# volume-em/empanada

Measured on AMD Instinct MI355X. Metric: Mvox/s end-to-end 3D panoptic inference (incl. consensus); PQ vs CPU ref, higher is better.
Workload: dtype f32

## Files before the change

### empanada_amd/_hip.py

```python
import ctypes
import os

import torch

_HERE = os.path.dirname(os.path.abspath(__file__))
LIB_PATH = os.path.join(_HERE, 'libemp_hip.so')

MAX_KS = 11
MAX_CLASSES = 16
MAX_CENTERS = 4096
CENTER_LIMIT = 65535


class HipError(RuntimeError):
    pass


_c = ctypes
_P = _c.c_void_p
_I = _c.c_int
_L = _c.c_int64
_F = _c.c_float
_U32 = _c.c_uint32

SIGNATURES = {
    'emp_version': (_I, []),
    'emp_last_error': (_c.c_char_p, []),
    'emp_device_count': (_I, []),
    'emp_bn_act_nhwc': (_I, [_P, _P, _P, _P, _I, _L, _I, _P, _L, _P]),
    'emp_dwconv_nhwc': (_I, [_P, _P, _P, _I, _I, _I, _I, _I, _P, _P]),
    'emp_upsample_bilinear': (_I, [_P, _I, _I, _I, _I, _P, _P, _I, _I, _P, _P]),
    'emp_conv_bn_act_proj_nhwc': (_I, [_P, _P, _P, _P, _I] + [_I] * 10 + [_P, _I, _P, _P, _L, _P]),
    'emp_conv_k_slab': (_I, [_L, _I, _I, _I]),
    'emp_conv_k_slab_cin': (_I, [_L, _I, _I, _I, _I]),
    'emp_conv_k_slab_geom': (_I, [_L, _I, _I, _I, _I, _I, _I, _I, _I]),
    'emp_conv1x1_ws_eligible': (_I, [_L, _I, _I, _I, _I, _I, _I, _I]),
    'emp_gconv_chunk': (_I, [_I]),
    'emp_gconv3x3_bn_act_nhwc': (_I, [_P, _L, _P, _P, _P, _I, _I, _I, _I, _I, _I, _I, _P, _L, _P]),
    'emp_conv_bn_act_nhwc': (_I, [_P, _P, _P, _P, _P, _L, _I] + [_I] * 10 + [_P, _L, _P]),
    'emp_conv_splitk_plan': (_I, [_L, _I, _I, _I, _I]),
    'emp_conv_splitk_bn_act_nhwc': (_I, [_P, _P, _P, _P, _P, _L, _I] + [_I] * 11 + [_P, _P, _L, _P]),
    'emp_wino_input_transform': (_I, [_P, _I, _I, _I, _I, _I, _P, _L, _P, _P]),
    'emp_gemm_nt_batched': (_I, [_P, _P, _I, _L, _I, _I, _P, _P]),
    'emp_wino4_input_transform': (_I, [_P, _I, _I, _I, _I, _I, _P, _L, _P, _P]),
    'emp_wino4_output_transform': (_I, [_P, _P, _L, _I, _I, _I, _I, _I, _P, _P, _I, _P, _L, _P]),
    'emp_wino4_conv_bn_act_nhwc': (_I, [_P, _I, _I, _I, _I, _I, _P, _L, _P, _I, _P, _P, _I, _P, _L, _P]),
    'emp_wino4_fused_eligible': (_I, [_L, _I, _I, _I]),
    'emp_wino3_input_transform': (_I, [_P, _I, _I, _I, _I, _I, _P, _L, _P, _P]),
    'emp_wino3_output_transform': (_I, [_P, _P, _L, _I, _I, _I, _I, _I, _P, _P, _I, _P, _L, _P]),
    'emp_wino_gemm_fused': (_I, [_P, _I, _I, _I, _I, _I, _P, _L, _P, _I, _P, _P]),
    'emp_wino_output_transform': (_I, [_P, _P, _L, _I, _I, _I, _I, _I, _P, _P, _I, _P, _L, _P]),
    'emp_chain_class': (_I, [_L, _P, _P, _P, _I, _P, _P, _P, _P, _L, _L, _c.c_double, _c.c_double, _P, _P, _P, _P]),
    'emp_lsap_maximize': (_L, [_P, _L, _L, _P, _P]),
    'emp_slices_to_input': (_I, [_P, _L, _L, _L, _I, _I, _I, _I, _I, _F, _F, _P, _P]),
    'emp_slices_to_input_scaled': (_I, [_P, _L, _L, _L] + [_I] * 7 + [_P, _P, _P, _P, _I, _F, _F, _P, _P]),
    'emp_pointwise_out_nhwc': (_I, [_P, _P, _P, _L, _L, _I, _I, _P, _P]),
    'emp_bn_relu_maxpool_nhwc': (_I, [_P, _P, _P, _I, _I, _I, _I, _P, _P]),
    'emp_stem_conv7_bn_relu_maxpool': (_I, [_P, _P, _P, _P, _I, _I, _I, _P, _P]),
    'emp_logits_to_prob': (_I, [_P, _I, _I, _L, _P, _P]),
    'emp_upsample_bilinear_prob': (_I, [_P, _I, _I, _I, _I, _P, _P, _I, _I, _P, _I, _P]),
    'emp_pr_upsample2x': (_I, [_P, _I, _I, _I, _I, _P, _P, _P]),
    'emp_pr_topk_work_bytes': (_L, [_I, _L]),
    'emp_pr_topk': (_I, [_P, _I, _L, _I, _P, _L, _P, _P]),
    'emp_pr_point_sample': (_I, [_P, _L, _P, _I, _I, _I, _I, _I, _P, _I, _I, _I, _P, _P, _I, _P]),
    'emp_pr_scatter': (_I, [_P, _I, _P, _I, _I, _I, _L, _P, _P]),
    'emp_median_harden_stack': (_I, [_P, _I, _I, _L, _I, _F, _P, _P, _P]),
    'emp_median_step': (_I, [_c.POINTER(_P), _I, _L, _P, _P]),
    'emp_harden': (_I, [_P, _I, _I, _L, _F, _P, _P]),
    'emp_find_centers': (_I, [_P, _I, _I, _I, _F, _I, _I, _P, _P, _P]),
    'emp_find_centers_work_elems': (_L, [_I, _I, _I, _I]),
    'emp_find_centers_ws': (_I, [_P, _I, _I, _I, _F, _I, _I, _P, _P, _P, _P]),
    'emp_group_work_elems': (_L, [_I, _I]),
    'emp_group_pixels': (_I, [_P, _P, _I, _P, _I, _I, _I, _I, _P, _U32, _P, _P, _P]),
    'emp_fuse_work_elems': (_L, [_I, _I, _I]),
    'emp_fuse_panoptic': (_I, [_P, _P, _I, _I, _I, _I, _I, _I, _U32, _L, _L, _L, _P, _P, _P, _P]),
    'emp_fuse_lut': (_I, [_P, _P, _I, _I, _I, _I, _I, _I, _U32, _L, _L, _P, _P]),
    'emp_fuse_apply': (_I, [_P, _P, _I, _I, _I, _I, _I, _I, _U32, _L, _L, _P, _P, _P, _P]),
    'emp_runs_count': (_I, [_P, _I, _I, _I, _P, _P]),
    'emp_scan_tmp_elems': (_L, [_L]),
    'emp_exclusive_scan_i32': (_I, [_P, _L, _P, _P, _P]),
    'emp_runs_extract': (_I, [_P, _I, _I, _I, _P, _P, _P, _P, _P]),
    'emp_runs_label_work_elems': (_L, [_L]),
    'emp_runs_label': (_I, [_P, _P, _P, _P, _L, _I, _I, _I, _L, _U32, _P, _P, _P, _P, _P, _P, _P, _P, _P]),
    'emp_runs_overlap_next': (_I, [_P, _P, _P, _P, _P, _L, _I, _I, _I, _L, _P, _L, _P, _P]),
    'emp_rle_decode': (_I, [_P, _P, _P, _L, _P, _P]),
# ... 854 lines not shown
    g = w_oihw.detach().double().cpu()

    def comb(a, b, c):
        return [(G[0] * a + G[1] * b) + G[2] * c for G in _WINO3_G]

    rows = comb(g[:, :, 0, :], g[:, :, 1, :], g[:, :, 2, :])
    U = []
    for r in rows:
        U.extend(comb(r[:, :, 0], r[:, :, 1], r[:, :, 2]))
    return torch.stack(U, dim=0).float().contiguous()


def wino3_conv_bn_act(x, U, tiles_dev, dil, scale=None, shift=None, relu=False, out=None):
    require_gpu()
    N, Cin, H, W = x.shape
    Cout = U.shape[1]
    assert x.is_cuda and x.dtype == torch.float32 and x.is_contiguous(memory_format=torch.channels_last)
    T = tiles_dev.shape[0]
    V = torch.empty((25, T, Cin), dtype=torch.float32, device=x.device)
    Mw = torch.empty((25, T, Cout), dtype=torch.float32, device=x.device)
    if out is None:
        out = torch.empty((N, Cout, H, W), dtype=torch.float32, device=x.device, memory_format=torch.channels_last)
    assert out.shape == (N, Cout, H, W) and out.stride(1) == 1
    ops = out.stride(3)
    assert out.stride(2) == W * ops and out.stride(0) == H * W * ops, "NHWC channel slice required"
    st = stream()
    call('emp_wino3_input_transform', x.data_ptr(), N, H, W, Cin, dil, _ptr(tiles_dev), T, _ptr(V), st,
         alg_bytes=4 * (x.numel() + V.numel()))
    call('emp_gemm_nt_batched', _ptr(V), _ptr(U), 25, T, Cout, Cin, _ptr(Mw), st,
         alg_bytes=4 * (V.numel() + U.numel() + Mw.numel()), alg_flops=2 * 25 * T * Cout * Cin)
    call('emp_wino3_output_transform', _ptr(Mw), _ptr(tiles_dev), T, N, H, W, Cout, dil, _ptr(scale), _ptr(shift),
         int(bool(relu)), out.data_ptr(), ops, st, alg_bytes=4 * (Mw.numel() + N * Cout * H * W))
    return out


def conv_bn_act_proj_nhwc(x, w_okkc, scale, shift, relu, proj_w, proj_b=None, stride=1, pad=0, dil=1, keep=False):
    require_gpu()
    N, Cin, H, W = x.shape
    Cout, KH, KW, _ = w_okkc.shape
    n = proj_w.shape[0]
    assert x.is_cuda and x.dtype == torch.float32 and x.is_contiguous(memory_format=torch.channels_last)
    OH = (H + 2 * pad - dil * (KH - 1) - 1) // stride + 1
    OW = (W + 2 * pad - dil * (KW - 1) - 1) // stride + 1
    acc = torch.zeros((N, n, OH, OW), dtype=torch.float32, device=x.device)
    act = (torch.empty((N, Cout, OH, OW), dtype=torch.float32, device=x.device, memory_format=torch.channels_last)
           if keep else None)
    call('emp_conv_bn_act_proj_nhwc', x.data_ptr(), _ptr(w_okkc), _ptr(scale), _ptr(shift), int(bool(relu)), N, H, W,
         Cin, Cout, KH, KW, stride, pad, dil, _ptr(proj_w), n, _ptr(acc), act.data_ptr() if keep else None, 0,
         stream(), alg_bytes=4 * (x.numel() + w_okkc.numel() + acc.numel() + (act.numel() if keep else 0)),
         alg_flops=2 * N * OH * OW * Cout * (Cin * KH * KW + n))
    if proj_b is not None:
        acc += proj_b.view(1, -1, 1, 1)
    return (acc, act) if keep else acc
```

### empanada_amd/build.py

```python
import os
import subprocess
import sys

HERE = os.path.dirname(os.path.abspath(__file__))
CSRC = os.path.join(HERE, 'csrc')
SOURCES = ['emp_pixel.hip', 'emp_runs.hip', 'emp_ranges.hip', 'emp_tracks.hip', 'emp_dense.hip', 'emp_conv.hip', 'emp_conv1x1.hip', 'emp_wino4.hip', 'emp_gconv.hip', 'emp_stem.hip', 'emp_pointrend.hip', 'emp_chain.cpp']
LIB = os.path.join(HERE, 'libemp_hip.so')
FLAGS = ['--offload-arch=gfx950', '-O3', '-ffp-contract=off', '-fPIC', '-std=c++17', '-Wno-unused-value',
         '-Wno-unused-result', '-Wno-inline-asm']


def _stale(target, deps):
    if not os.path.exists(target):
        return True
    t = os.path.getmtime(target)
    return any(os.path.getmtime(d) > t for d in deps)


def build(force=False, verbose=True):
    hipcc = os.environ.get('HIPCC', 'hipcc')
    headers = [os.path.join(CSRC, 'emp_common.h'), os.path.join(CSRC, 'emp_wino4.h'), os.path.join(HERE, '..', 'include', 'emp_hip.h')]
    objs = []
    for src in SOURCES:
        s = os.path.join(CSRC, src)
        o = os.path.join(CSRC, os.path.splitext(src)[0] + '.o')
        if force or _stale(o, [s] + headers):
            cmd = [hipcc] + FLAGS + ['-c', s, '-o', o]
            if verbose:
                print(' '.join(cmd), flush=True)
            subprocess.run(cmd, check=True)
        objs.append(o)
    if force or _stale(LIB, objs):
        cmd = [hipcc, '--offload-arch=gfx950', '-shared', '-fPIC', '-o', LIB] + objs
        if verbose:
            print(' '.join(cmd), flush=True)
        subprocess.run(cmd, check=True)
    return LIB


if __name__ == '__main__':
    build(force='--force' in sys.argv)
```

### empanada_amd/csrc/emp_conv.hip

```cpp
#include "emp_common.h"
#include "emp_wino4.h"
#include <stdlib.h>

typedef float f32x16 __attribute__((ext_vector_type(16)));

#define CG_BM 128
#define CG_BK 32
#define CG_THREADS 256

struct ConvGeom {
    const float *x, *w, *scale, *shift, *res;
    float *out;
    int N, H, W, Cin, OH, OW, Cout, KH, KW, stride, pad, dil, relu;
    int64_t M, out_ps, res_ps;
    int tiles_m, tiles_n;
    int64_t x_bs, w_bs, out_bs;
    const int32_t *tiles;
    const float *proj_w;
    float *proj_out;
    int proj_n;
    int64_t hw;
};

__device__ __attribute__((aligned(16))) float cg_zero_page[64];
// ... 653 lines not shown
    const int T = g.tiles_m * g.tiles_n;
    const dim3 grid(8 * ((T + 7) / 8), 1, k_splits);
    hipStream_t st = emp_stream(stream);
    if (pl.narrow)
        hipLaunchKernelGGL((conv_igemm_f32_kernel<1, 0, false, 32, false, true>), grid, dim3(CG_THREADS), 0, st, g);
    else
        hipLaunchKernelGGL((conv_igemm_f32_kernel<2, 0, false, 32, false, true>), grid, dim3(CG_THREADS), 0, st, g);
    EMP_CHECK_LAUNCH("emp_conv_splitk_bn_act_nhwc(partials)");
    const int64_t total = g.M * (Cout / 4);
    hipLaunchKernelGGL(splitk_reduce_kernel, dim3(emp_grid(total, 256, 4096)), dim3(256), 0, st, work, k_splits, g.M, Cout,
                       scale, shift, residual, res_pixel_stride, relu, out, out_pixel_stride);
    EMP_CHECK_LAUNCH("emp_conv_splitk_bn_act_nhwc(reduce)");
    return EMP_OK;
}

extern "C" int emp_conv_bn_act_proj_nhwc(const float *x, const float *w_okkc, const float *scale, const float *shift,
                                         int relu, int N, int H, int W, int Cin, int Cout, int KH, int KW, int stride,
                                         int pad, int dil, const float *proj_w, int proj_n, float *proj_out,
                                         float *out, int64_t out_pixel_stride, void *stream)
{
    EMP_REQUIRE(x && w_okkc && proj_w && proj_out, "conv_proj: null pointer");
    EMP_REQUIRE(N >= 0 && H > 0 && W > 0 && Cin > 0 && Cin % CG_BK == 0, "conv_proj: bad shape (Cin %% %d)", CG_BK);
    EMP_REQUIRE(Cout == 128 || Cout == 256, "conv_proj: Cout %d must be 128 or 256 (at most two cout tiles)", Cout);
    EMP_REQUIRE(proj_n >= 1 && proj_n <= 4, "conv_proj: proj_n %d not in 1..4", proj_n);
    EMP_REQUIRE(KH >= 1 && KW >= 1 && KH <= 7 && KW <= 7 && stride >= 1 && dil >= 1 && pad >= 0, "conv_proj: bad filter geometry");
    const int OH = (H + 2 * pad - dil * (KH - 1) - 1) / stride + 1;
    const int OW = (W + 2 * pad - dil * (KW - 1) - 1) / stride + 1;
    EMP_REQUIRE(OH > 0 && OW > 0, "conv_proj: empty output");
    if (out_pixel_stride == 0) out_pixel_stride = Cout;
    EMP_REQUIRE(((reinterpret_cast<uintptr_t>(x) | reinterpret_cast<uintptr_t>(w_okkc) | reinterpret_cast<uintptr_t>(proj_w) |
                  reinterpret_cast<uintptr_t>(out)) & 15) == 0 && (out_pixel_stride & 3) == 0, "conv_proj: alignment");
    EMP_REQUIRE(out != x, "conv_proj: output cannot alias the input");
    if (N == 0) return EMP_OK;
    ConvGeom g;
    g.x = x; g.w = w_okkc; g.scale = scale; g.shift = shift; g.res = nullptr; g.out = out;
    g.N = N; g.H = H; g.W = W; g.Cin = Cin; g.OH = OH; g.OW = OW; g.Cout = Cout; g.KH = KH; g.KW = KW;
    g.stride = stride; g.pad = pad; g.dil = dil; g.relu = relu;
    g.M = (int64_t)N * OH * OW; g.out_ps = out_pixel_stride; g.res_ps = Cout;
    g.x_bs = g.w_bs = g.out_bs = 0; g.tiles = nullptr;
    g.proj_w = proj_w; g.proj_out = proj_out; g.proj_n = proj_n; g.hw = (int64_t)OH * OW;
    const CgPlan pl = cg_plan(g.M, Cout, 1, false, true, false);
    g.tiles_m = pl.tiles_m;
    g.tiles_n = pl.tiles_n;
    const int T = g.tiles_m * g.tiles_n;
    const int grid = 8 * ((T + 7) / 8);
#define CG_GOP(BK_, GL_) hipLaunchKernelGGL((conv_igemm_f32_kernel<2, 0, false, BK_, true, GL_>), dim3(grid), dim3(CG_THREADS), 0, emp_stream(stream), g)
    if (pl.glds) { if (pl.slab == 16) CG_GOP(16, true); else CG_GOP(32, true); }
    else { if (pl.slab == 16) CG_GOP(16, false); else CG_GOP(32, false); }
#undef CG_GOP
    EMP_CHECK_LAUNCH("emp_conv_bn_act_proj_nhwc");
    return EMP_OK;
}


__global__ __launch_bounds__(256) void wino_input_kernel(const float *__restrict__ x, const int32_t *__restrict__ tiles,
                                                         int64_t T, int H, int W, int C4, int dil, float4 *__restrict__ V)
{
    const int64_t total = T * C4;
    for (int64_t i = (int64_t)blockIdx.x * blockDim.x + threadIdx.x; i < total; i += (int64_t)gridDim.x * blockDim.x) {
        const int c4 = (int)(i % C4);
        const int64_t t = i / C4;
        const int n = tiles[3 * t], by = tiles[3 * t + 1], bx = tiles[3 * t + 2];
        const float4 *src = reinterpret_cast<const float4 *>(x) + (int64_t)n * H * W * C4 + c4;
        float4 d[4][4];
#pragma unroll
        for (int a = 0; a < 4; ++a)
#pragma unroll
            for (int b = 0; b < 4; ++b) {
                const int yy = by + a * dil, xx = bx + b * dil;
                d[a][b] = make_float4(0.f, 0.f, 0.f, 0.f);
                if (yy >= 0 && yy < H && xx >= 0 && xx < W) d[a][b] = src[((int64_t)yy * W + xx) * C4];
            }
#define W_SUB(p, q) make_float4(__fsub_rn(p.x, q.x), __fsub_rn(p.y, q.y), __fsub_rn(p.z, q.z), __fsub_rn(p.w, q.w))
#define W_ADD(p, q) make_float4(__fadd_rn(p.x, q.x), __fadd_rn(p.y, q.y), __fadd_rn(p.z, q.z), __fadd_rn(p.w, q.w))
        float4 tt[4][4];
#pragma unroll
        for (int a = 0; a < 4; ++a) {
            tt[a][0] = W_SUB(d[a][0], d[a][2]);
            tt[a][1] = W_ADD(d[a][1], d[a][2]);
            tt[a][2] = W_SUB(d[a][2], d[a][1]);
            tt[a][3] = W_SUB(d[a][1], d[a][3]);
        }
        float4 *dst = V + t * C4 + c4;
        const int64_t ps = T * C4;
#pragma unroll
        for (int v = 0; v < 4; ++v) {
            dst[(0 * 4 + v) * ps] = W_SUB(tt[0][v], tt[2][v]);
            dst[(1 * 4 + v) * ps] = W_ADD(tt[1][v], tt[2][v]);
            dst[(2 * 4 + v) * ps] = W_SUB(tt[2][v], tt[1][v]);
            dst[(3 * 4 + v) * ps] = W_SUB(tt[1][v], tt[3][v]);
        }
    }
}

__global__ __launch_bounds__(256) void wino_output_kernel(const float4 *__restrict__ Mw, const int32_t *__restrict__ tiles,
                                                          int64_t T, int H, int W, int Co4, int dil,
                                                          const float4 *__restrict__ scale, const float4 *__restrict__ shift,
                                                          int relu, float *__restrict__ out, int64_t out_ps)
{
    const int64_t total = T * Co4;
    for (int64_t i = (int64_t)blockIdx.x * blockDim.x + threadIdx.x; i < total; i += (int64_t)gridDim.x * blockDim.x) {
        const int c4 = (int)(i % Co4);
        const int64_t t = i / Co4;
        const int n = tiles[3 * t], oy = tiles[3 * t + 1] + dil, ox = tiles[3 * t + 2] + dil;
        const float4 *src = Mw + t * Co4 + c4;
        const int64_t ps = T * Co4;
// ... 385 lines not shown
```

### empanada_amd/models/panoptic_deeplab.py

```python
import zlib
from typing import List

import torch
import torch.nn as nn
import torch.nn.functional as F

__all__ = ['PanopticDeepLab', 'PanopticDeepLabPR', 'PointRendSemSegHead', 'resnet_encoder', 'prepare_for_inference',
           'tune_fused_convs',
           'synthesize_weights']

_RESNETS = {
    'resnet18': ('basic', [2, 2, 2, 2]), 'resnet34': ('basic', [3, 4, 6, 3]),
    'resnet50': ('bottleneck', [3, 4, 6, 3]), 'resnet101': ('bottleneck', [3, 4, 23, 3]),
    'resnet152': ('bottleneck', [3, 8, 36, 3]),
}


def _conv_bn_act(nin, nout, k, stride=1, groups=1, act=True):
    layers = [nn.Conv2d(nin, nout, k, stride=stride, padding=(k - 1) // 2, groups=groups, bias=False),
              nn.BatchNorm2d(nout)]
    if act:
        layers.append(nn.ReLU(inplace=True))
    return nn.Sequential(*layers)


class SeparableConv2d(nn.Module):

    def __init__(self, nin, nout, kernel_size=3, stride=1, bias=True):
        super().__init__()
        self.sepconv = nn.Sequential(
            nn.Conv2d(nin, nin, kernel_size, stride=stride, padding=(kernel_size - 1) // 2, groups=nin, bias=bias),
            nn.Conv2d(nin, nout, 1, stride=1, bias=bias))

    def forward(self, x):
        return self.sepconv(x)


def _sepconv_bn_act(nin, nout, k):
    return nn.Sequential(SeparableConv2d(nin, nout, k, 1, bias=False), nn.BatchNorm2d(nout), nn.ReLU(inplace=True))


def _bn_affine(bn):
    scale = (bn.weight.detach().float() / torch.sqrt(bn.running_var.detach().float() + bn.eps)).contiguous()
    shift = (bn.bias.detach().float() - bn.running_mean.detach().float() * scale).contiguous()
    return scale, shift


def _no_late_weights(state_dict, prefix, *args):
    raise RuntimeError("load_state_dict after prepare_for_inference: load the weights into the plain model first "
                       f"(module {prefix.rstrip('.')!r} holds folded copies)")


class DepthwiseConvNHWC(nn.Module):

    def __init__(self, conv):
        super().__init__()
        k = conv.kernel_size[0]
        C = conv.in_channels
        self.register_buffer('w_kkc', conv.weight.detach().float().reshape(C, k * k).t().contiguous())
        self.register_buffer('b', conv.bias.detach().float().contiguous() if conv.bias is not None else None)
        self.k = k

    @staticmethod
    def eligible(m):
        return (isinstance(m, nn.Conv2d) and m.groups == m.in_channels == m.out_channels and m.in_channels % 4 == 0
                and m.kernel_size[0] == m.kernel_size[1] and m.kernel_size[0] in (3, 5) and m.stride == (1, 1)
                and m.dilation == (1, 1) and m.padding == (m.kernel_size[0] // 2,) * 2
                and m.padding_mode == 'zeros')

    def forward(self, x):
        from .. import _hip
        if not x.is_contiguous(memory_format=torch.channels_last):
            x = x.contiguous(memory_format=torch.channels_last)
        return _hip.dwconv_nhwc(x, self.w_kkc, self.b, self.k)


class FusedBNAct(nn.Module):

    def __init__(self, bn, relu):
        super().__init__()
        scale, shift = _bn_affine(bn)
        self.register_buffer('scale', scale, persistent=False)
        self.register_buffer('shift', shift, persistent=False)
        self.relu = relu
        self._register_load_state_dict_pre_hook(_no_late_weights)

    def forward(self, x, residual=None, out=None):
        from .. import _hip
# ... 331 lines not shown
        return self.project(torch.cat([conv(x) for conv in self.convs], dim=1))


class PanopticDeepLabDecoder(nn.Module):

    def __init__(self, in_channels, decoder_channels, low_level_stages, low_level_channels,
                 low_level_channels_project, atrous_rates, aspp_channels=None, aspp_dropout=0.5):
        super().__init__()
        aspp_channels = aspp_channels or decoder_channels
        self.aspp = ASPP(in_channels, aspp_channels, atrous_rates, aspp_dropout)
        self.low_level_stages = list(low_level_stages)
        project, fuse = [], []
        for i, (lc, pc) in enumerate(zip(low_level_channels, low_level_channels_project)):
            project.append(_conv_bn_act(lc, pc, 1))
            fuse.append(_sepconv_bn_act((aspp_channels if i == 0 else decoder_channels) + pc, decoder_channels, 5))
        self.project = nn.ModuleList(project)
        self.fuse = nn.ModuleList(fuse)
        self.hip_ops = False

    def forward(self, pyramid: List[torch.Tensor]):
        x = self.aspp(pyramid[-1])
        for stage, proj, fuse in zip(self.low_level_stages, self.project, self.fuse):
            feat = pyramid[stage]
            if self.hip_ops and _can_write_into(proj, feat):
                cx = x.shape[1]
                cl = (proj[0].conv if isinstance(proj[0], FusedConvBNAct) else proj[0]).out_channels
                buf = torch.empty((x.shape[0], cx + cl, feat.shape[2], feat.shape[3]), dtype=x.dtype,
                                  device=x.device, memory_format=torch.channels_last)
                _up_bilinear(x, feat.shape[2:], True, out=buf[:, :cx])
                _conv_bn_into(proj, feat, buf[:, cx:])
                x = fuse(buf)
            else:
                low = proj(feat)
                x = _up_bilinear(x, low.shape[2:], self.hip_ops)
                x = fuse(torch.cat((x, low), dim=1))
        return x


class PanopticDeepLabHead(nn.Module):

    def __init__(self, nin, n_classes):
        super().__init__()
        self.head = nn.Sequential(_sepconv_bn_act(nin, nin, 5), nn.Conv2d(nin, n_classes, 1, bias=True))
        self.hip_ops = False

    def forward(self, x):
        if self.hip_ops and x.is_cuda and x.dtype == torch.float32:
            sep = self.head[0][0]
            site = sep.sepconv[1] if isinstance(sep, SeparableConv2d) else None
            last = self.head[1]
            if (isinstance(site, FusedConvBNAct) and site.impl == 'direct' and isinstance(last, PointwiseOutNHWC)
                    and site.conv.out_channels in (128, 256) and site.conv.kernel_size == (1, 1)):
                from .. import _hip
                y = sep.sepconv[0](x)
                if not y.is_contiguous(memory_format=torch.channels_last):
                    y = y.contiguous(memory_format=torch.channels_last)
                site._prepare('direct')
                return _hip.conv_bn_act_proj_nhwc(y, site._w_okkc, site.bn.scale, site.bn.shift, site.bn.relu,
                                                  last.w, last.b)
        return self.head(x)


class PanopticDeepLab(nn.Module):

    def __init__(self, encoder='resnet50', num_classes=1, stage4_stride=16, decoder_channels=256,
                 low_level_stages=(3, 2, 1), low_level_channels_project=(128, 64, 32), atrous_rates=(2, 4, 6),
                 aspp_channels=None, aspp_dropout=0.1, ins_decoder=False, ins_ratio=0.5, **kwargs):
        super().__init__()
        assert encoder in _RESNETS, f'Invalid encoder name {encoder}, choices are {sorted(_RESNETS)}'
        assert stage4_stride in (16, 32) and min(low_level_stages) > 0
        self.decoder_channels = decoder_channels
        self.num_classes = num_classes
        self.encoder = resnet_encoder(encoder, output_stride=stage4_stride)
        sem_p, ins_p = (aspp_dropout, aspp_dropout) if isinstance(aspp_dropout, float) else aspp_dropout
        widths = self.encoder.cfg.widths
        low_ch = [int(widths[i - 1]) for i in low_level_stages]
        self.semantic_decoder = PanopticDeepLabDecoder(int(widths[-1]), decoder_channels, low_level_stages, low_ch,
                                                       list(low_level_channels_project), atrous_rates,
                                                       aspp_channels, sem_p)
        if ins_decoder:
            self.instance_decoder = PanopticDeepLabDecoder(
                int(widths[-1]), decoder_channels, low_level_stages, low_ch,
                [int(s * ins_ratio) for s in low_level_channels_project], atrous_rates, aspp_channels, ins_p)
        else:
            self.instance_decoder = None
        self.semantic_head = PanopticDeepLabHead(decoder_channels, num_classes)
        self.ins_center = PanopticDeepLabHead(decoder_channels, 1)
        self.ins_xy = PanopticDeepLabHead(decoder_channels, 2)

    hip_ops = False

    def _up4(self, x):
        return _up_bilinear(x, (4 * x.shape[2], 4 * x.shape[3]), self.hip_ops)

    defer_up4 = False

    def _finish(self, heads, up):
        if not self.defer_up4:
            return {k: self._up4(v) if k in up else v for k, v in heads.items()}
        return dict(heads, deferred_up4=tuple(up))

    def forward(self, x):
        pyramid = self.encoder(x)
        sem_x = self.semantic_decoder(pyramid)
        ins_x = sem_x if self.instance_decoder is None else self.instance_decoder(pyramid)
        return self._finish({'sem_logits': self.semantic_head(sem_x), 'ctr_hmp': self.ins_center(ins_x),
                             'offsets': self.ins_xy(ins_x)}, ('sem_logits', 'ctr_hmp', 'offsets'))
# ... 253 lines not shown
```

### include/emp_hip.h

```cpp
#ifndef EMP_HIP_H
#define EMP_HIP_H

#include <stdint.h>

#ifdef __cplusplus
extern "C" {
#endif

#define EMP_OK 0
#define EMP_EINVAL (-1)
#define EMP_ELAUNCH (-2)
#define EMP_ENODEV (-3)

#define EMP_MAX_KS 11
#define EMP_MAX_CLASSES 16
#define EMP_MAX_CENTERS 4096
#define EMP_CENTER_LIMIT 65535

int emp_version(void);
const char *emp_last_error(void);
int emp_device_count(void);

int emp_slices_to_input(const uint8_t *vol, int64_t stride_slice, int64_t stride_row, int64_t stride_col,
                        int n_slices, int h, int w, int hp, int wp, float mean255, float inv_std255,
                        float *out, void *stream);

int emp_slices_to_input_scaled(const uint8_t *vol, int64_t stride_slice, int64_t stride_row, int64_t stride_col,
                               int n_slices, int h, int w, int dh, int dw, int hp, int wp, const int32_t *row_off,
                               const int16_t *row_coef, const int32_t *col_off, const int16_t *col_coef, int area,
                               float mean255, float inv_std255, float *out, void *stream);

int emp_bn_act_nhwc(const float *x, const float *scale, const float *shift, const float *residual,
                    int relu, int64_t n_pixels, int C, float *out, int64_t out_pixel_stride, void *stream);

int emp_dwconv_nhwc(const float *x, const float *w_kkc, const float *bias, int N, int H, int W, int C,
                    int k, float *y, void *stream);

int emp_upsample_bilinear(const float *x, int N, int C, int h, int w, const int64_t *x_strides,
                          float *y, int H, int W, const int64_t *y_strides, void *stream);

int emp_conv_k_slab(int64_t M, int Cout, int batch, int has_residual);
int emp_conv_k_slab_cin(int64_t M, int Cout, int batch, int has_residual, int Cin);
int emp_conv_k_slab_geom(int64_t M, int Cout, int has_residual, int Cin, int KH, int KW, int stride, int pad, int relu);
int emp_conv1x1_ws_eligible(int64_t M, int Cin, int Cout, int KH, int KW, int stride, int pad, int relu);
int emp_conv_bn_act_nhwc(const float *x, const float *w_okkc, const float *scale, const float *shift,
                         const float *residual, int64_t res_pixel_stride, int relu, int N, int H, int W,
                         int Cin, int Cout, int KH, int KW, int stride, int pad, int dil, float *out,
                         int64_t out_pixel_stride, void *stream);
int emp_conv_splitk_plan(int64_t M, int Cout, int Cin, int KH, int KW);
int emp_conv_splitk_bn_act_nhwc(const float *x, const float *w_okkc, const float *scale, const float *shift,
                                const float *residual, int64_t res_pixel_stride, int relu, int N, int H, int W,
                                int Cin, int Cout, int KH, int KW, int stride, int pad, int dil, int k_splits,
                                float *work, float *out, int64_t out_pixel_stride, void *stream);

int emp_conv_bn_act_proj_nhwc(const float *x, const float *w_okkc, const float *scale, const float *shift,
                              int relu, int N, int H, int W, int Cin, int Cout, int KH, int KW, int stride,
                              int pad, int dil, const float *proj_w, int proj_n, float *proj_out,
                              float *out, int64_t out_pixel_stride, void *stream);

int emp_gconv_chunk(int group_w);
int emp_gconv3x3_bn_act_nhwc(const float *x, int64_t x_pixel_stride, const float *w_okkc, const float *scale,
                             const float *shift, int relu, int N, int H, int W, int groups, int group_w,
                             int stride, float *out, int64_t out_pixel_stride, void *stream);

int emp_wino_input_transform(const float *x, int N, int H, int W, int C, int dil, const int32_t *tiles,
                             int64_t T, float *V, void *stream);
int emp_gemm_nt_batched(const float *A, const float *B, int batch, int64_t M, int N, int K, float *C,
                        void *stream);
int emp_wino_gemm_fused(const float *x, int N, int H, int W, int Cin, int dil, const int32_t *tiles,
                        int64_t T, const float *U, int Cout, float *Mw, void *stream);
int emp_wino_output_transform(const float *Mw, const int32_t *tiles, int64_t T, int N, int H, int W,
                              int Cout, int dil, const float *scale, const float *shift, int relu,
                              float *out, int64_t out_pixel_stride, void *stream);

int emp_wino4_input_transform(const float *x, int N, int H, int W, int C, int dil, const int32_t *tiles,
                              int64_t T, float *V, void *stream);
int emp_wino4_output_transform(const float *Mw, const int32_t *tiles, int64_t T, int N, int H, int W,
                               int Cout, int dil, const float *scale, const float *shift, int relu,
                               float *out, int64_t out_pixel_stride, void *stream);
int emp_wino4_conv_bn_act_nhwc(const float *x, int N, int H, int W, int Cin, int dil, const int32_t *tiles, int64_t T,
                               const float *U, int Cout, const float *scale, const float *shift, int relu,
                               float *out, int64_t out_pixel_stride, void *stream);
int emp_wino4_fused_eligible(int64_t T, int Cin, int Cout, int has_scale_shift);

int emp_wino3_input_transform(const float *x, int N, int H, int W, int C, int dil, const int32_t *tiles,
                              int64_t T, float *V, void *stream);
int emp_wino3_output_transform(const float *Mw, const int32_t *tiles, int64_t T, int N, int H, int W,
                               int Cout, int dil, const float *scale, const float *shift, int relu,
                               float *out, int64_t out_pixel_stride, void *stream);

int emp_pointwise_out_nhwc(const float *x, const float *w, const float *bias, int64_t n_pixels,
                           int64_t pixels_per_image, int C, int Cout, float *out, void *stream);

int emp_bn_relu_maxpool_nhwc(const float *x, const float *scale, const float *shift, int N, int H, int W,
                             int C, float *y, void *stream);

int emp_stem_conv7_bn_relu_maxpool(const float *x, const float *w_tc, const float *scale, const float *shift,
                                   int N, int H, int W, float *y, void *stream);

int emp_logits_to_prob(const float *logits, int N, int C, int64_t HW, float *prob, void *stream);

int emp_upsample_bilinear_prob(const float *x, int N, int C, int h, int w, const int64_t *x_strides,
                               float *y, int H, int W, const int64_t *y_strides, int prob, void *stream);

int emp_median_harden_stack(const float *prob, int D, int C, int64_t HW, int ks, float thr,
                            uint8_t *out_sem, float *out_prob, void *stream);

int emp_median_step(const float *const *slices_host, int ks, int64_t n, float *out, void *stream);

int emp_harden(const float *prob, int D, int C, int64_t HW, float thr, uint8_t *out_sem,
               void *stream);
// ... 126 lines not shown
```

Measured before the change: 131.9.

## Fuse depthwise 5x5 and pointwise 1x1 conv into one MFMA kernel

Adds a fused separable-convolution kernel. It computes the 5x5 depthwise conv on a haloed input patch held in LDS, writes the result straight into the A-tile of an MFMA GEMM against the pointwise weights, and applies BN scale/shift, ReLU and an optional small projection head in the epilogue. Input loads are double-buffered with global-to-LDS loads. This removes the round trip of the depthwise intermediate through global memory and one launch per separable-conv site in the decoder heads. The cost is a larger, more specialised kernel that only covers Cout=256, k=5 and a few Cin values, with its own eligibility gate and an env switch to turn it off.

After: 131.8, median of 3. About the same (-0.0%).

```diff
diff --git a/empanada_amd/_hip.py b/empanada_amd/_hip.py
--- a/empanada_amd/_hip.py
+++ b/empanada_amd/_hip.py
@@ -31,6 +31,9 @@
     'emp_dwconv_nhwc': (_I, [_P, _P, _P, _I, _I, _I, _I, _I, _P, _P]),
     'emp_upsample_bilinear': (_I, [_P, _I, _I, _I, _I, _P, _P, _I, _I, _P, _P]),
     'emp_conv_bn_act_proj_nhwc': (_I, [_P, _P, _P, _P, _I] + [_I] * 10 + [_P, _I, _P, _P, _L, _P]),
+    'emp_sepconv_bn_act_nhwc': (_I, [_P, _P, _P, _I, _P, _P, _P, _I, _I, _I, _I, _I, _I, _P, _L, _P]),
+    'emp_sepconv_bn_act_proj_nhwc': (_I, [_P, _P, _P, _I, _P, _P, _P, _I, _I, _I, _I, _I, _I, _P, _P, _I, _P, _P, _L, _P]),
+    'emp_sepconv_eligible': (_I, [_L, _I, _I, _I, _I, _I, _I]),
     'emp_conv_k_slab': (_I, [_L, _I, _I, _I]),
     'emp_conv_k_slab_cin': (_I, [_L, _I, _I, _I, _I]),
     'emp_conv_k_slab_geom': (_I, [_L, _I, _I, _I, _I, _I, _I, _I, _I]),
@@ -991,3 +994,50 @@
     if proj_b is not None:
         acc += proj_b.view(1, -1, 1, 1)
     return (acc, act) if keep else acc
+
+
+def sepconv_eligible(M, Cin, Cout, k, has_scale_shift=True, proj=False, relu=True):
+    return bool(load().emp_sepconv_eligible(int(M), int(Cin), int(Cout), int(k), int(bool(has_scale_shift)),
+                                            int(bool(proj)), int(bool(relu))))
+
+
+def _sepconv_args(x, dw_kkc, dw_bias, w_okkc, scale, shift):
+    N, Cin, H, W = x.shape
+    assert x.is_cuda and x.dtype == torch.float32 and x.is_contiguous(memory_format=torch.channels_last)
+    k = int(round(dw_kkc.shape[0] ** 0.5))
+    for what, t, numel in (("depthwise table", dw_kkc, None), ("pointwise filter", w_okkc, None),
+                           ("depthwise bias", dw_bias, Cin), ("scale", scale, w_okkc.shape[0]), ("shift", shift, w_okkc.shape[0])):
+        if t is not None:
+            _expect(f"sepconv: {what}", t, torch.float32, numel=numel)
+    if tuple(dw_kkc.shape) != (k * k, Cin) or w_okkc.numel() != w_okkc.shape[0] * Cin or w_okkc.shape[-1] != Cin:
+        raise HipError(f"sepconv: depthwise table {tuple(dw_kkc.shape)} / pointwise filter {tuple(w_okkc.shape)} do not "
+                       f"match {Cin} input channels")
+    return N, Cin, H, W, k, w_okkc.shape[0]
+
+
+def sepconv_bn_act(x, dw_kkc, dw_bias, w_okkc, scale, shift, relu, out=None):
+    require_gpu()
+    N, Cin, H, W, k, Cout = _sepconv_args(x, dw_kkc, dw_bias, w_okkc, scale, shift)
+    if out is None:
+        out = torch.empty((N, Cout, H, W), dtype=torch.float32, device=x.device, memory_format=torch.channels_last)
+    assert out.shape == (N, Cout, H, W) and out.stride(1) == 1
+    ops = out.stride(3)
+    assert out.stride(2) == W * ops and out.stride(0) == H * W * ops, "NHWC channel slice required"
+    call('emp_sepconv_bn_act_nhwc', x.data_ptr(), _ptr(dw_kkc), _ptr(dw_bias), k, _ptr(w_okkc), _ptr(scale), _ptr(shift),
+         int(bool(relu)), N, H, W, Cin, Cout, out.data_ptr(), ops, stream(), profile_as='emp_conv_bn_act_nhwc',
+         alg_bytes=4 * (x.numel() + w_okkc.numel() + N * Cout * H * W), alg_flops=2 * N * H * W * Cin * (Cout + k * k))
+    return out
+
+
+def sepconv_bn_act_proj(x, dw_kkc, dw_bias, w_okkc, scale, shift, relu, proj_w, proj_b=None):
+    require_gpu()
+    N, Cin, H, W, k, Cout = _sepconv_args(x, dw_kkc, dw_bias, w_okkc, scale, shift)
+    n = proj_w.shape[0]
+    if tuple(proj_w.shape) != (n, Cout) or (proj_b is not None and proj_b.numel() != n):
+        raise HipError(f"sepconv_proj: projection {tuple(proj_w.shape)} does not match {Cout} channels")
+    res = torch.empty((N, n, H, W), dtype=torch.float32, device=x.device)
+    call('emp_sepconv_bn_act_proj_nhwc', x.data_ptr(), _ptr(dw_kkc), _ptr(dw_bias), k, _ptr(w_okkc), _ptr(scale),
+         _ptr(shift), int(bool(relu)), N, H, W, Cin, Cout, _ptr(proj_w), _ptr(proj_b), n, res.data_ptr(), None, 0, stream(),
+         profile_as='emp_conv_bn_act_proj_nhwc', alg_bytes=4 * (x.numel() + w_okkc.numel() + res.numel()),
+         alg_flops=2 * N * H * W * (Cin * (Cout + k * k) + Cout * n))
+    return res
diff --git a/empanada_amd/build.py b/empanada_amd/build.py
--- a/empanada_amd/build.py
+++ b/empanada_amd/build.py
@@ -4,7 +4,7 @@
 
 HERE = os.path.dirname(os.path.abspath(__file__))
 CSRC = os.path.join(HERE, 'csrc')
-SOURCES = ['emp_pixel.hip', 'emp_runs.hip', 'emp_ranges.hip', 'emp_tracks.hip', 'emp_dense.hip', 'emp_conv.hip', 'emp_conv1x1.hip', 'emp_wino4.hip', 'emp_gconv.hip', 'emp_stem.hip', 'emp_pointrend.hip', 'emp_chain.cpp']
+SOURCES = ['emp_pixel.hip', 'emp_runs.hip', 'emp_ranges.hip', 'emp_tracks.hip', 'emp_dense.hip', 'emp_conv.hip', 'emp_conv1x1.hip', 'emp_wino4.hip', 'emp_sepconv.hip', 'emp_gconv.hip', 'emp_stem.hip', 'emp_pointrend.hip', 'emp_chain.cpp']
 LIB = os.path.join(HERE, 'libemp_hip.so')
 FLAGS = ['--offload-arch=gfx950', '-O3', '-ffp-contract=off', '-fPIC', '-std=c++17', '-Wno-unused-value',
          '-Wno-unused-result', '-Wno-inline-asm']
diff --git a/empanada_amd/csrc/emp_conv.hip b/empanada_amd/csrc/emp_conv.hip
--- a/empanada_amd/csrc/emp_conv.hip
+++ b/empanada_amd/csrc/emp_conv.hip
@@ -729,6 +729,11 @@
     return EMP_OK;
 }
 
+extern "C" __attribute__((visibility("hidden"))) int emp_conv_proj_k_slab(int64_t M, int Cout)
+{
+    return cg_plan(M, Cout, 1, false, true, false).slab;
+}
+
 
 __global__ __launch_bounds__(256) void wino_input_kernel(const float *__restrict__ x, const int32_t *__restrict__ tiles,
                                                          int64_t T, int H, int W, int C4, int dil, float4 *__restrict__ V)
diff --git a/empanada_amd/csrc/emp_sepconv.hip b/empanada_amd/csrc/emp_sepconv.hip
--- /dev/null
+++ b/empanada_amd/csrc/emp_sepconv.hip
@@ -0,0 +1,337 @@
+#include "emp_common.h"
+#include <stdlib.h>
+
+typedef float f32x16 __attribute__((ext_vector_type(16)));
+
+#define SC_THREADS 256
+#define SC_TH 8
+#define SC_TW 16
+#define SC_BM (SC_TH * SC_TW)
+#define SC_COUT 256
+#define SC_BK 16
+#define SC_PW (SC_TW + 4)
+#define SC_PH (SC_TH + 4)
+#define SC_PPIX 256
+#define SC_EROWS 32
+#define SC_CLD (SC_COUT + 4)
+
+struct SepGeom {
+    const float *x, *dw, *dwb, *w, *scale, *shift, *proj_w, *proj_b;
+    float *out, *proj_out;
+    int N, H, W, Cin, relu, proj_n;
+    int64_t out_ps;
+    int gx, gy, total;
+};
+
+__device__ __attribute__((aligned(16))) float sc_zero_page[16];
+
+__device__ __forceinline__ void sc_glds16(const float *src, unsigned lds_byte_addr)
+{
+    asm volatile("s_mov_b32 m0, %1\n\ts_nop 0\n\tglobal_load_lds_dwordx4 %0, off" ::"v"(src), "s"(lds_byte_addr) : "memory", "m0");
+}
+
+__device__ __forceinline__ void sc_wait_vm0()
+{
+    asm volatile("s_waitcnt vmcnt(0)" ::: "memory");
+}
+
+typedef float sc_v4 __attribute__((ext_vector_type(4)));
+typedef const __attribute__((address_space(4))) sc_v4 sc_cf4;
+
+template <bool PROJ>
+__global__ __launch_bounds__(SC_THREADS, 2) void sepconv_fused_kernel(SepGeom g)
+{
+    constexpr int P_ELEMS = SC_PPIX * SC_BK, A_ELEMS = SC_BM * SC_BK, B_ELEMS = SC_COUT * SC_BK;
+    constexpr int SMEM = 2 * (P_ELEMS + A_ELEMS + B_ELEMS);
+    static_assert(SMEM >= SC_EROWS * SC_CLD, "epilogue staging fits the K-loop buffers");
+    __shared__ __attribute__((aligned(16))) float smem[SMEM];
+    float *Ps = smem, *As = smem + 2 * P_ELEMS, *Bs = smem + 2 * (P_ELEMS + A_ELEMS);
+
+    const int chunk = (g.total + 7) >> 3;
+    const int tile = (blockIdx.x & 7) * chunk + (blockIdx.x >> 3);
+    if (tile >= g.total) return;
+    const int bx = tile % g.gx, by = (tile / g.gx) % g.gy, n = tile / (g.gx * g.gy);
+    const int x0 = bx * SC_TW, y0 = by * SC_TH;
+
+    const int tid = threadIdx.x;
+    const int wave = __builtin_amdgcn_readfirstlane(tid >> 6), lane = tid & 63;
+    const int wm = wave >> 1, wn = wave & 1;
+    const int r = lane & 31, hh = lane >> 5;
+
+    const unsigned lds0 = (unsigned)(size_t)(__attribute__((address_space(3))) float *)smem;
+    int p_off[4];
+#pragma unroll
+    for (int k = 0; k < 4; ++k) {
+        const int f = k * SC_THREADS + tid;
+        const int pp = f >> 2;
+        const int py = pp / SC_PW, px = pp - py * SC_PW;
+        const int lc = (f & 3) ^ ((px >> 2) & 3);
+        const int iy = y0 - 2 + py, ix = x0 - 2 + px;
+        const bool ok = pp < SC_PH * SC_PW && iy >= 0 && iy < g.H && ix >= 0 && ix < g.W;
+        p_off[k] = ok ? (((n * g.H + iy) * g.W + ix) * g.Cin + lc * 4) : -1;
+    }
+    const float *b_src = g.w + (int64_t)(tid >> 2) * g.Cin + (((tid & 3) ^ ((tid >> 4) & 3)) * 4);
+    const int64_t b_step = (int64_t)64 * g.Cin;
+    const unsigned wl = (unsigned)(wave * 64 * 16);
+    const unsigned p_dst = __builtin_amdgcn_readfirstlane(lds0 + wl);
+    const unsigned b_dst = __builtin_amdgcn_readfirstlane(lds0 + (unsigned)(2 * (P_ELEMS + A_ELEMS) * 4) + wl);
+    auto issue_patch = [&](int s, int buf) {
+#pragma unroll
+        for (int k = 0; k < 4; ++k) {
+            const float *src = p_off[k] >= 0 ? g.x + p_off[k] + s * SC_BK : sc_zero_page;
+            sc_glds16(src, p_dst + (unsigned)((buf * P_ELEMS + k * SC_THREADS * 4) * 4));
+        }
+    };
+    auto issue_b = [&](int s, int buf) {
+#pragma unroll
+        for (int k = 0; k < 4; ++k) sc_glds16(b_src + k * b_step + s * SC_BK, b_dst + (unsigned)((buf * B_ELEMS + k * SC_THREADS * 4) * 4));
+    };
+
+    const int dcol = lane & 15, drow = 2 * (((lane >> 4) & 1) * 2 + (lane >> 5));
+    float4 dbias = make_float4(0.f, 0.f, 0.f, 0.f);
+    auto depthwise = [&](int s, int buf) {
+        sc_cf4 *wq = reinterpret_cast<sc_cf4 *>(reinterpret_cast<uintptr_t>(g.dw + s * SC_BK + wave * 4));
+        const int wst = g.Cin >> 2;
+        if (g.dwb) {
+            const sc_v4 b4 = *reinterpret_cast<sc_cf4 *>(reinterpret_cast<uintptr_t>(g.dwb + s * SC_BK + wave * 4));
+            dbias = make_float4(b4.x, b4.y, b4.z, b4.w);
+        }
+        const float *Pb = Ps + buf * P_ELEMS;
+        float4 o0 = make_float4(0.f, 0.f, 0.f, 0.f), o1 = o0;
+#pragma unroll
+        for (int ir = 0; ir < 6; ++ir) {
+            float4 in[5];
+#pragma unroll
+            for (int j = 0; j < 5; ++j) {
+                const int pp = (drow + ir) * SC_PW + dcol + j;
+                in[j] = *reinterpret_cast<const float4 *>(Pb + pp * SC_BK + ((wave ^ (((dcol + j) >> 2) & 3)) * 4));
+            }
+            if (ir < 5) {
+#pragma unroll
+                for (int j = 0; j < 5; ++j) {
+                    const sc_v4 wt = wq[(ir * 5 + j) * wst];
+                    o0.x = fmaf(in[j].x, wt.x, o0.x); o0.y = fmaf(in[j].y, wt.y, o0.y);
+                    o0.z = fmaf(in[j].z, wt.z, o0.z); o0.w = fmaf(in[j].w, wt.w, o0.w);
+                }
+            }
+            if (ir >= 1) {
+#pragma unroll
+                for (int j = 0; j < 5; ++j) {
+                    const sc_v4 wt = wq[((ir - 1) * 5 + j) * wst];
+                    o1.x = fmaf(in[j].x, wt.x, o1.x); o1.y = fmaf(in[j].y, wt.y, o1.y);
+                    o1.z = fmaf(in[j].z, wt.z, o1.z); o1.w = fmaf(in[j].w, wt.w, o1.w);
+                }
+            }
+            __builtin_amdgcn_sched_barrier(0);
+        }
+        o0.x = __fadd_rn(o0.x, dbias.x); o0.y = __fadd_rn(o0.y, dbias.y); o0.z = __fadd_rn(o0.z, dbias.z); o0.w = __fadd_rn(o0.w, dbias.w);
+        o1.x = __fadd_rn(o1.x, dbias.x); o1.y = __fadd_rn(o1.y, dbias.y); o1.z = __fadd_rn(o1.z, dbias.z); o1.w = __fadd_rn(o1.w, dbias.w);
+        const int m0 = drow * SC_TW + dcol, m1 = m0 + SC_TW;
+        float *Ab = As + buf * A_ELEMS;
+        *reinterpret_cast<float4 *>(Ab + m0 * SC_BK + ((wave ^ ((m0 >> 2) & 3)) * 4)) = o0;
+        *reinterpret_cast<float4 *>(Ab + m1 * SC_BK + ((wave ^ ((m1 >> 2) & 3)) * 4)) = o1;
+    };
+
+    f32x16 acc[2][4];
+#pragma unroll
+    for (int i = 0; i < 2; ++i)
+#pragma unroll
+        for (int j = 0; j < 4; ++j)
+#pragma unroll
+            for (int q = 0; q < 16; ++q) acc[i][j][q] = 0.f;
+
+    const int S = g.Cin / SC_BK;
+    const int swz_rd = (r >> 2) & 3;
+
+    issue_patch(0, 0);
+    issue_b(0, 0);
+    sc_wait_vm0();
+    __builtin_amdgcn_s_barrier();
+    if (S > 1) issue_patch(1, 1);
+    depthwise(0, 0);
+    sc_wait_vm0();
+    __syncthreads();
+    for (int s = 0; s < S; ++s) {
+        const int buf = s & 1;
+        if (s + 1 < S) issue_b(s + 1, buf ^ 1);
+        if (s + 2 < S) issue_patch(s + 2, buf);
+        if (s + 1 < S) depthwise(s + 1, buf ^ 1);
+        const float *Ar = As + buf * A_ELEMS + (wm * 64 + r) * SC_BK;
+        const float *Br = Bs + buf * B_ELEMS + (wn * 128 + r) * SC_BK;
+#pragma unroll
+        for (int f = 0; f < 2; ++f) {
+            const int pc = ((hh * 2 + f) ^ swz_rd) * 4;
+            float4 fa[2], fb[4];
+#pragma unroll
+            for (int i = 0; i < 2; ++i) fa[i] = *reinterpret_cast<const float4 *>(Ar + i * 32 * SC_BK + pc);
+#pragma unroll
+            for (int j = 0; j < 4; ++j) fb[j] = *reinterpret_cast<const float4 *>(Br + j * 32 * SC_BK + pc);
+#pragma unroll
+            for (int e = 0; e < 4; ++e) {
+                float av[2], bv[4];
+#pragma unroll
+                for (int i = 0; i < 2; ++i) av[i] = e == 0 ? fa[i].x : e == 1 ? fa[i].y : e == 2 ? fa[i].z : fa[i].w;
+#pragma unroll
+                for (int j = 0; j < 4; ++j) bv[j] = e == 0 ? fb[j].x : e == 1 ? fb[j].y : e == 2 ? fb[j].z : fb[j].w;
+#pragma unroll
+                for (int i = 0; i < 2; ++i)
+#pragma unroll
+                    for (int j = 0; j < 4; ++j)
+                        acc[i][j] = __builtin_amdgcn_mfma_f32_32x32x2f32(av[i], bv[j], acc[i][j], 0, 0, 0);
+            }
+        }
+        sc_wait_vm0();
+        __syncthreads();
+    }
+
+    float *Cs = smem;
+    const int ccol = (tid & 63) * 4, crow = tid >> 6;
+    const float4 sc4 = *reinterpret_cast<const float4 *>(g.scale + ccol);
+    const float4 sh4 = *reinterpret_cast<const float4 *>(g.shift + ccol);
+    const float sc[4] = {sc4.x, sc4.y, sc4.z, sc4.w}, sh[4] = {sh4.x, sh4.y, sh4.z, sh4.w};
+    const int64_t hw = (int64_t)g.H * g.W;
+#pragma unroll
+    for (int rd = 0; rd < SC_BM / SC_EROWS; ++rd) {
+        if (rd > 0) __syncthreads();
+        if (wm == (rd >> 1)) {
+#pragma unroll
+            for (int j = 0; j < 4; ++j)
+#pragma unroll
+                for (int q = 0; q < 16; ++q) {
+                    const int row = (q & 3) + 8 * (q >> 2) + 4 * hh;
+                    Cs[row * SC_CLD + wn * 128 + j * 32 + r] = acc[rd & 1][j][q];
+                }
+        }
+        __syncthreads();
+#pragma unroll
+        for (int it = 0; it < SC_EROWS / 4; ++it) {
+            const int lrow = crow + 4 * it, m = rd * SC_EROWS + lrow;
+            const int oy = y0 + (m >> 4), ox = x0 + (m & 15);
+            const bool valid = oy < g.H && ox < g.W;
+            float v[4] = {0.f, 0.f, 0.f, 0.f};
+            if (valid) {
+                const float4 a4 = *reinterpret_cast<const float4 *>(&Cs[lrow * SC_CLD + ccol]);
+                v[0] = a4.x; v[1] = a4.y; v[2] = a4.z; v[3] = a4.w;
+#pragma unroll
+                for (int e = 0; e < 4; ++e) v[e] = __fadd_rn(__fmul_rn(v[e], sc[e]), sh[e]);
+                if (g.relu) {
+#pragma unroll
+                    for (int e = 0; e < 4; ++e) v[e] = fmaxf(v[e], 0.f);
+                }
+                if (!PROJ || g.out)
+                    *reinterpret_cast<float4 *>(g.out + ((int64_t)n * hw + (int64_t)oy * g.W + ox) * g.out_ps + ccol) =
+                        make_float4(v[0], v[1], v[2], v[3]);
+            }
+            if constexpr (PROJ) {
+                float ps[4] = {0.f, 0.f, 0.f, 0.f};
+                if (valid) {
+#pragma unroll
+                    for (int q = 0; q < 4; ++q)
+                        if (q < g.proj_n) {
+                            const float4 wq = *reinterpret_cast<const float4 *>(g.proj_w + q * SC_COUT + ccol);
+                            ps[q] = __fadd_rn(__fadd_rn(__fadd_rn(__fmul_rn(v[0], wq.x), __fmul_rn(v[1], wq.y)),
+                                                        __fmul_rn(v[2], wq.z)), __fmul_rn(v[3], wq.w));
+                        }
+                }
+                *reinterpret_cast<float4 *>(&Cs[lrow * SC_CLD + ccol]) = make_float4(ps[0], ps[1], ps[2], ps[3]);
+            }
+        }
+        if constexpr (PROJ) {
+            __syncthreads();
+            for (int idx = tid; idx < SC_EROWS * g.proj_n; idx += SC_THREADS) {
+                const int row_l = idx / g.proj_n, q = idx - row_l * g.proj_n;
+                const int m = rd * SC_EROWS + row_l;
+                const int oy = y0 + (m >> 4), ox = x0 + (m & 15);
+                if (oy < g.H && ox < g.W) {
+                    float total = 0.f;
+#pragma unroll
+                    for (int h = 0; h < 2; ++h) {
+                        float t = Cs[row_l * SC_CLD + h * 128 + q];
+#pragma unroll 8
+                        for (int j = 1; j < 32; ++j) t = __fadd_rn(t, Cs[row_l * SC_CLD + h * 128 + 4 * j + q]);
+                        total = __fadd_rn(total, t);
+                    }
+                    if (g.proj_b) total = __fadd_rn(total, g.proj_b[q]);
+                    g.proj_out[((int64_t)n * g.proj_n + q) * hw + (int64_t)oy * g.W + ox] = total;
+                }
+            }
+        }
+    }
+}
+
+extern "C" __attribute__((visibility("hidden"))) int emp_conv_proj_k_slab(int64_t M, int Cout);
+
+static bool sc_off()
+{
+    static const char *off = getenv("EMP_SEPCONV_NO_FUSED");
+    return off && off[0] == '1';
+}
+
+static bool sc_shape_ok(int64_t M, int Cin, int Cout, int k, int proj, int relu)
+{
+    if (k != 5 || Cin <= 0 || Cin % SC_BK != 0 || Cout != SC_COUT || M <= 0) return false;
+    if (M * (int64_t)Cin >= (1LL << 31)) return false;
+    if (proj) return Cin % 32 == 0 && emp_conv_proj_k_slab(M, Cout) == SC_BK;
+    return emp_conv_k_slab_geom(M, Cout, 0, Cin, 1, 1, 1, 0, relu) == SC_BK;
+}
+
+extern "C" int emp_sepconv_eligible(int64_t M, int Cin, int Cout, int k, int has_scale_shift, int proj, int relu)
+{
+    if (sc_off() || !has_scale_shift) return 0;
+    if (!(Cin == 256 || Cin == 288 || Cin == 384)) return 0;
+    return sc_shape_ok(M, Cin, Cout, k, proj, relu) ? 1 : 0;
+}
+
+static int sc_launch(const float *x, const float *dw_kkc, const float *dw_bias, int k, const float *w_oc, const float *scale,
+                     const float *shift, int relu, int N, int H, int W, int Cin, int Cout, const float *proj_w,
+                     const float *proj_b, int proj_n, float *proj_out, float *out, int64_t out_ps, void *stream,
+                     const char *name)
+{
+    const bool proj = proj_out != nullptr;
+    EMP_REQUIRE(x && dw_kkc && w_oc && scale && shift, "%s: null pointer (scale and shift are required)", name);
+    EMP_REQUIRE(N >= 0 && H > 0 && W > 0, "%s: bad shape", name);
+    if (out_ps == 0) out_ps = Cout;
+    EMP_REQUIRE(out_ps >= Cout && (out_ps & 3) == 0, "%s: bad pixel stride", name);
+    EMP_REQUIRE(((reinterpret_cast<uintptr_t>(x) | reinterpret_cast<uintptr_t>(dw_kkc) | reinterpret_cast<uintptr_t>(dw_bias) |
+                  reinterpret_cast<uintptr_t>(w_oc) | reinterpret_cast<uintptr_t>(scale) | reinterpret_cast<uintptr_t>(shift) |
+                  reinterpret_cast<uintptr_t>(out) | reinterpret_cast<uintptr_t>(proj_w)) & 15) == 0, "%s: alignment", name);
+    EMP_REQUIRE(out != x, "%s: output cannot alias the input", name);
+    if (N == 0) return EMP_OK;
+    const int64_t M = (int64_t)N * H * W;
+    EMP_REQUIRE(sc_shape_ok(M, Cin, Cout, k, proj, relu),
+                "%s: depthwise 5x5, Cin %% 16 == 0, Cout == 256 and the K-slab 16 plan only (M = %lld, %d -> %d, k = %d)", name,
+                (long long)M, Cin, Cout, k);
+    SepGeom g;
+    g.x = x; g.dw = dw_kkc; g.dwb = dw_bias; g.w = w_oc; g.scale = scale; g.shift = shift;
+    g.proj_w = proj_w; g.proj_b = proj_b; g.out = out; g.proj_out = proj_out;
+    g.N = N; g.H = H; g.W = W; g.Cin = Cin; g.relu = relu; g.proj_n = proj_n; g.out_ps = out_ps;
+    g.gx = (int)emp_cdiv(W, SC_TW); g.gy = (int)emp_cdiv(H, SC_TH);
+    const int64_t total = (int64_t)g.gx * g.gy * N;
+    EMP_REQUIRE(total < (1LL << 28), "%s: too many tiles", name);
+    g.total = (int)total;
+    const dim3 grid(8 * ((g.total + 7) / 8)), block(SC_THREADS);
+    if (proj) hipLaunchKernelGGL((sepconv_fused_kernel<true>), grid, block, 0, emp_stream(stream), g);
+    else hipLaunchKernelGGL((sepconv_fused_kernel<false>), grid, block, 0, emp_stream(stream), g);
+    EMP_CHECK_LAUNCH(name);
+    return EMP_OK;
+}
+
+extern "C" int emp_sepconv_bn_act_nhwc(const float *x, const float *dw_kkc, const float *dw_bias, int k, const float *w_oc,
+                                       const float *scale, const float *shift, int relu, int N, int H, int W, int Cin,
+                                       int Cout, float *out, int64_t out_pixel_stride, void *stream)
+{
+    EMP_REQUIRE(out, "sepconv: null pointer");
+    return sc_launch(x, dw_kkc, dw_bias, k, w_oc, scale, shift, relu, N, H, W, Cin, Cout, nullptr, nullptr, 0, nullptr, out,
+                     out_pixel_stride, stream, "emp_sepconv_bn_act_nhwc");
+}
+
+extern "C" int emp_sepconv_bn_act_proj_nhwc(const float *x, const float *dw_kkc, const float *dw_bias, int k,
+                                            const float *w_oc, const float *scale, const float *shift, int relu, int N,
+                                            int H, int W, int Cin, int Cout, const float *proj_w, const float *proj_b,
+                                            int proj_n, float *proj_out, float *out, int64_t out_pixel_stride, void *stream)
+{
+    EMP_REQUIRE(proj_w && proj_out, "sepconv_proj: null pointer");
+    EMP_REQUIRE(proj_n >= 1 && proj_n <= 4, "sepconv_proj: proj_n %d not in 1..4", proj_n);
+    return sc_launch(x, dw_kkc, dw_bias, k, w_oc, scale, shift, relu, N, H, W, Cin, Cout, proj_w, proj_b, proj_n, proj_out,
+                     out, out_pixel_stride, stream, "emp_sepconv_bn_act_proj_nhwc");
+}
diff --git a/empanada_amd/models/panoptic_deeplab.py b/empanada_amd/models/panoptic_deeplab.py
--- a/empanada_amd/models/panoptic_deeplab.py
+++ b/empanada_amd/models/panoptic_deeplab.py
@@ -33,7 +33,23 @@
             nn.Conv2d(nin, nout, 1, stride=1, bias=bias))
 
     def forward(self, x):
+        dw, site = self.sepconv[0], self.sepconv[1]
+        if (isinstance(dw, DepthwiseConvNHWC) and isinstance(site, FusedConvBNAct) and site.impl == 'direct'
+                and x.is_cuda and x.dtype == torch.float32 and _is_plain_1x1(site.conv)):
+            from .. import _hip
+            N, C, H, W = x.shape
+            if _hip.sepconv_eligible(N * H * W, C, site.conv.out_channels, dw.k, True, False, site.bn.relu):
+                if not x.is_contiguous(memory_format=torch.channels_last):
+                    x = x.contiguous(memory_format=torch.channels_last)
+                site._seen = (tuple(x.shape), False)
+                site._prepare('direct')
+                return _hip.sepconv_bn_act(x, dw.w_kkc, dw.b, site._w_okkc, site.bn.scale, site.bn.shift, site.bn.relu)
         return self.sepconv(x)
+
+
+def _is_plain_1x1(conv):
+    return (conv.kernel_size == (1, 1) and conv.stride == (1, 1) and conv.padding == (0, 0) and conv.groups == 1
+            and conv.bias is None)
 
 
 def _sepconv_bn_act(nin, nout, k):
@@ -471,7 +487,16 @@
             if (isinstance(site, FusedConvBNAct) and site.impl == 'direct' and isinstance(last, PointwiseOutNHWC)
                     and site.conv.out_channels in (128, 256) and site.conv.kernel_size == (1, 1)):
                 from .. import _hip
-                y = sep.sepconv[0](x)
+                dw = sep.sepconv[0]
+                if (isinstance(dw, DepthwiseConvNHWC) and _is_plain_1x1(site.conv) and _hip.sepconv_eligible(
+                        x.shape[0] * x.shape[2] * x.shape[3], x.shape[1], site.conv.out_channels, dw.k, True, True,
+                        site.bn.relu)):
+                    if not x.is_contiguous(memory_format=torch.channels_last):
+                        x = x.contiguous(memory_format=torch.channels_last)
+                    site._prepare('direct')
+                    return _hip.sepconv_bn_act_proj(x, dw.w_kkc, dw.b, site._w_okkc, site.bn.scale, site.bn.shift,
+                                                    site.bn.relu, last.w, last.b)
+                y = dw(x)
                 if not y.is_contiguous(memory_format=torch.channels_last):
                     y = y.contiguous(memory_format=torch.channels_last)
                 site._prepare('direct')
diff --git a/include/emp_hip.h b/include/emp_hip.h
--- a/include/emp_hip.h
+++ b/include/emp_hip.h
@@ -57,6 +57,15 @@
                               int relu, int N, int H, int W, int Cin, int Cout, int KH, int KW, int stride,
                               int pad, int dil, const float *proj_w, int proj_n, float *proj_out,
                               float *out, int64_t out_pixel_stride, void *stream);
+
+int emp_sepconv_bn_act_nhwc(const float *x, const float *dw_kkc, const float *dw_bias, int k, const float *w_oc,
+                            const float *scale, const float *shift, int relu, int N, int H, int W, int Cin, int Cout,
+                            float *out, int64_t out_pixel_stride, void *stream);
+int emp_sepconv_bn_act_proj_nhwc(const float *x, const float *dw_kkc, const float *dw_bias, int k, const float *w_oc,
+                                 const float *scale, const float *shift, int relu, int N, int H, int W, int Cin,
+                                 int Cout, const float *proj_w, const float *proj_bias, int proj_n, float *proj_out,
+                                 float *out, int64_t out_pixel_stride, void *stream);
+int emp_sepconv_eligible(int64_t M, int Cin, int Cout, int k, int has_scale_shift, int proj, int relu);
 
 int emp_gconv_chunk(int group_w);
 int emp_gconv3x3_bn_act_nhwc(const float *x, int64_t x_pixel_stride, const float *w_okkc, const float *scale,
```
